# aclyde11/molecular-VAE

Measured on AMD Instinct MI355X. Metric: molecules/s (ELBO fwd+bwd+step), higher is better.
Workload: dtype bf16

## Files before the change

molecular-vae_amd/csrc/gemm.hip:

```cpp
#include "tile_pipe.hpp"
#include "kernels.hpp"
#include <stdlib.h>

struct GemmArgs {
  const void* A; const void* B; void* C; const float* bias; float* partial;
  long lda, ldb, ldc;
  int M, N, K;
  int c_dtype, act, accumulate;
  int tiles_m, tiles_n, splits;
  long kper;
  int a_group, b_group;
  long a_gstride, b_gstride, a_total, b_total;
  float* colsum_out; float* colsum_partial; int colsum_acc; int colsum_nparts; int ones_col;
};
__device__ __forceinline__ long grow(int r, int group, long gstride, long ld) {
  return group > 0 ? (long)(r / group) * gstride + (long)(r % group) * ld : (long)r * ld;
}

__device__ __forceinline__ void store_out(void* C, long off, int c_dtype, float v, int accumulate) {
  if (c_dtype == MVAE_F32) {
    float* p = reinterpret_cast<float*>(C) + off;
    *p = accumulate ? (*p + v) : v;
  } else {
    reinterpret_cast<bf16_t*>(C)[off].x = f2bf(v);
  }
}

__device__ __forceinline__ int xcd_remap(int bid, int n) {
  const int q = n >> 3, r = n & 7, x = bid & 7, i = bid >> 3;
  return (x < r ? x * (q + 1) : r * (q + 1) + (x - r) * q) + i;
}

template <typename T, int BM, int BN, bool PIPE, bool X3 = false>
__global__ __launch_bounds__(256) void gemm_nt_kernel(GemmArgs p) {
  extern __shared__ __attribute__((aligned(16))) char smem[];
  constexpr int WM = BM / 2, WN = BN / 2, MI = WM / 16, NI = WN / 16;
  const int tid = threadIdx.x, lane = tid & 63, wave = tid >> 6, wm = wave >> 1, wn = wave & 1;
  const int ntile = p.tiles_m * p.tiles_n;
  const int tile = xcd_remap(blockIdx.x, ntile);
  const int tm = tile / p.tiles_n, tn = tile - tm * p.tiles_n;
  const int m0 = tm * BM, n0 = tn * BN;
  const int split = blockIdx.y;
  const long kbeg = (long)split * p.kper;
  const long kend = (kbeg + p.kper < (long)p.K) ? (kbeg + p.kper) : (long)p.K;

  const T* A = reinterpret_cast<const T*>(p.A);
  const T* B = reinterpret_cast<const T*>(p.B);
  auto rowA = [&](int r) -> const T* { const int gm = m0 + r; return gm < p.M ? A + grow(gm, p.a_group, p.a_gstride, p.lda) : nullptr; };
  auto rowB = [&](int r) -> const T* { const int gn = n0 + r; return gn < p.N ? B + (long)gn * p.ldb : nullptr; };

  f32x4 acc[MI][NI];
#pragma unroll
  for (int i = 0; i < MI; ++i)
#pragma unroll
    for (int j = 0; j < NI; ++j) acc[i][j] = f32x4{0.f, 0.f, 0.f, 0.f};
  int brow[NI];
#pragma unroll
  for (int j = 0; j < NI; ++j) brow[j] = wn * WN + j * 16;

  if constexpr (PIPE) {
    constexpr int NBUF = 4;
    PipeSeg<BM, BN> s0, s1;
    const uint32_t sz = (uint32_t)sizeof(T);
    auto offA = [&](int r) -> uint32_t { const int gm = m0 + r; return gm < p.M ? (uint32_t)grow(gm, p.a_group, p.a_gstride, p.lda) * sz : PIPE_OOB; };
    auto offB = [&](int r) -> uint32_t { const int gn = n0 + r; return gn < p.N ? (uint32_t)gn * (uint32_t)p.ldb * sz : PIPE_OOB; };
    const uint32_t bytesA = (uint32_t)(p.a_total * sz - kbeg * sz), bytesB = (uint32_t)((long)p.N * p.ldb * sz - kbeg * sz);
    pipe_seg_init<T, BM, BN>(s0, A + kbeg, bytesA, B + kbeg, bytesB, offA, offB, (int)(kend - kbeg), tid);
    s1 = s0; s1.nk = 0;
    tile_gemm_pipe<T, BM, BN, MI, NI, NBUF, NI, 0, X3>(smem, s0, s1, wm * WM, wn * WN, acc, tid);
  } else {
    tile_gemm_segment<T, BM, BN, MI, NI>(smem, rowA, rowB, kbeg, kend, wm * WM, brow, acc, tid);
  }

  const int lr = lane & 15, lq = lane >> 4;
#pragma unroll
  for (int i = 0; i < MI; ++i)
#pragma unroll
    for (int j = 0; j < NI; ++j) {
      const int col = n0 + wn * WN + j * 16 + lr;
      if (col >= p.N) continue;
#pragma unroll
      for (int r = 0; r < 4; ++r) {
        const int row = m0 + wm * WM + i * 16 + lq * 4 + r;
        if (row >= p.M) continue;
        float v = acc[i][j][r];
        if (p.splits > 1) {
          p.partial[((long)split * p.M + row) * p.N + col] = v;
        } else {
          if (p.bias) v += p.bias[col];
          if (p.act == MVAE_ACT_SELU) v = selu_f(v); else if (p.act == MVAE_ACT_RELU) v = fmaxf(v, 0.f);
          store_out(p.C, (long)row * p.ldc + col, p.c_dtype, v, p.accumulate);
        }
      }
    }
}

__global__ __launch_bounds__(256) void gemm_splitk_reduce_kernel(GemmArgs p) {
  const long n = (long)p.M * p.N;
  for (long i = (long)blockIdx.x * 256 + threadIdx.x; i < n; i += (long)gridDim.x * 256) {
    const int row = (int)(i / p.N), col = (int)(i - (long)row * p.N);
    float v = 0.f;
    for (int s = 0; s < p.splits; ++s) v += p.partial[(long)s * n + i];
    if (p.bias) v += p.bias[col];
    if (p.act == MVAE_ACT_SELU) v = selu_f(v); else if (p.act == MVAE_ACT_RELU) v = fmaxf(v, 0.f);
    store_out(p.C, (long)row * p.ldc + col, p.c_dtype, v, p.accumulate);
  }
  if (p.colsum_out && p.colsum_partial) {
    for (long i = (long)blockIdx.x * 256 + threadIdx.x; i < p.M; i += (long)gridDim.x * 256) {
// ... 158 lines not shown
  }
}
struct TnColsumFinish { const float* partial[MVAE_MAX_LAYERS * 2]; float* out[MVAE_MAX_LAYERS * 2]; int M[MVAE_MAX_LAYERS * 2], acc[MVAE_MAX_LAYERS * 2]; int n; };
__global__ __launch_bounds__(256) void gemm_tn_colsum_finish_kernel(TnColsumFinish f) {
  const int gi = blockIdx.y;
  if (gi >= f.n) return;
  for (int i = blockIdx.x * 256 + threadIdx.x; i < f.M[gi]; i += gridDim.x * 256) {
    const float v = f.partial[gi][i] + f.partial[gi][f.M[gi] + i];
    f.out[gi][i] = f.acc[gi] ? f.out[gi][i] + v : v;
  }
}

namespace {
struct Plan { int bm, bn, tiles_m, tiles_n, splits; long kper; };

Plan make_plan(int M, int N, int K, int dtype) {
  Plan pl;
  const int ke = (dtype == MVAE_BF16) ? 64 : 32;
  const long t128 = (long)((M + 127) / 128) * ((N + 127) / 128), t64 = (long)((M + 63) / 64) * ((N + 63) / 64);
  auto eff = [](long t) { return (double)t / (double)(((t + 255) / 256) * 256); };
  pl.bm = (t128 >= 192 && eff(t128) >= 0.8 * eff(t64)) ? 128 : 64;
  pl.bn = pl.bm;
  if (dtype == MVAE_F32 && N <= 32 && M >= 128) { pl.bm = 128; pl.bn = 32; }
  pl.tiles_m = (M + pl.bm - 1) / pl.bm;
  pl.tiles_n = (N + pl.bn - 1) / pl.bn;
  const long tiles = (long)pl.tiles_m * pl.tiles_n;
  long ksteps = (K + ke - 1) / ke;
  if (ksteps < 1) ksteps = 1;
  int splits = 1;
  if (tiles < 128 && ksteps >= 16) {
    splits = (int)((256 + tiles - 1) / tiles);
    const long maxs = ksteps / 8;
    if (splits > maxs) splits = (int)maxs;
    if (splits > 64) splits = 64;
    if (splits < 1) splits = 1;
  }
  long per = (ksteps + splits - 1) / splits;
  splits = (int)((ksteps + per - 1) / per);
  pl.splits = splits;
  pl.kper = per * ke;
  return pl;
}
}

size_t gemm_nt_workspace_bytes(int M, int N, int K, int dtype) {
  if (dtype == MVAE_F32X3) dtype = MVAE_F32;
  Plan pl = make_plan(M, N, K, dtype);
  return pl.splits > 1 ? (size_t)pl.splits * M * N * sizeof(float) : 0;
}

int launch_gemm_nt(int dtype, int M, int N, int K, const void* A, long lda, const void* B, long ldb, void* C, long ldc,
                   int c_dtype, const float* bias, int act, int accumulate, void* ws, size_t ws_bytes, hipStream_t st) {
  return launch_gemm_nt_grouped(dtype, M, N, K, A, lda, 0, 0, (long)M * lda, B, ldb, C, ldc, c_dtype, bias, act, accumulate, ws, ws_bytes, st);
}

int launch_gemm_nt_grouped(int dtype, int M, int N, int K, const void* A, long lda, int a_group, long a_gstride, long a_total,
                           const void* B, long ldb, void* C, long ldc, int c_dtype, const float* bias, int act, int accumulate,
                           void* ws, size_t ws_bytes, hipStream_t st) {
  if (M <= 0 || N <= 0) return MVAE_OK;
  if (K < 0 || !A || !B || !C) return MVAE_ERR_INVALID;
  const bool x3 = dtype == MVAE_F32X3;
  if (x3) dtype = MVAE_F32;
  if (dtype != MVAE_F32 && dtype != MVAE_BF16) return MVAE_ERR_INVALID;
  if (c_dtype != MVAE_F32 && c_dtype != MVAE_BF16) return MVAE_ERR_INVALID;
  if (accumulate && c_dtype != MVAE_F32) return MVAE_ERR_INVALID;
  Plan pl = make_plan(M, N, K, dtype);
  GemmArgs p;
  p.A = A; p.B = B; p.C = C; p.bias = bias; p.partial = nullptr;
  p.lda = lda; p.ldb = ldb; p.ldc = ldc; p.M = M; p.N = N; p.K = K;
  p.c_dtype = c_dtype; p.act = act; p.accumulate = accumulate;
  p.tiles_m = pl.tiles_m; p.tiles_n = pl.tiles_n; p.splits = pl.splits; p.kper = pl.kper;
  p.a_group = a_group; p.a_gstride = a_gstride; p.a_total = a_total; p.b_group = 0; p.b_gstride = 0; p.b_total = (long)N * ldb;
  p.colsum_out = nullptr; p.colsum_partial = nullptr; p.colsum_acc = 0; p.colsum_nparts = 0; p.ones_col = -1;
  if (pl.splits > 1) {
    const size_t need = (size_t)pl.splits * M * N * sizeof(float);
    if (!ws || ws_bytes < need) return MVAE_ERR_WORKSPACE;
    p.partial = reinterpret_cast<float*>(ws);
  }
  dim3 grid(pl.tiles_m * pl.tiles_n, pl.splits), block(256);
  const int sz = (dtype == MVAE_BF16) ? 2 : 4, ke = KB / sz;
  const bool pipe = (K % ke == 0) && (pl.kper % ke == 0) && (lda % (16 / sz) == 0) && (ldb % (16 / sz) == 0) &&
                    ((reinterpret_cast<uintptr_t>(A) | reinterpret_cast<uintptr_t>(B)) % 16 == 0) &&
                    (a_total * sz < (1L << 31)) && ((long)N * ldb * sz < (1L << 31)) && K >= 4 * ke &&
                    (a_group == 0 || a_gstride % (16 / sz) == 0);
  const size_t lds = (size_t)(pipe ? 4 : 2) * (pl.bm + pl.bn) * KB;
#define MVAE_GEMM_LAUNCH2(TT_, BM_, BN_, PIPE_)                                                       \
  do {                                                                                                \
    auto kern = gemm_nt_kernel<TT_, BM_, BN_, PIPE_>;                                                 \
    static bool attr_set = false;                                                                     \
    if (!attr_set) { MVAE_CHECK_HIP(hipFuncSetAttribute(reinterpret_cast<const void*>(kern), hipFuncAttributeMaxDynamicSharedMemorySize, 160 * 1024)); attr_set = true; } \
    hipLaunchKernelGGL(kern, grid, block, lds, st, p);                                                \
  } while (0)
#define MVAE_GEMM_LAUNCH(TT_, BM_, PIPE_) MVAE_GEMM_LAUNCH2(TT_, BM_, BM_, PIPE_)
#define MVAE_GEMM_LAUNCH3(BM_)                                                                        \
  do {                                                                                                \
    auto kern = gemm_nt_kernel<float, BM_, BM_, true, true>;                                          \
    static bool attr_set = false;                                                                     \
    if (!attr_set) { MVAE_CHECK_HIP(hipFuncSetAttribute(reinterpret_cast<const void*>(kern), hipFuncAttributeMaxDynamicSharedMemorySize, 160 * 1024)); attr_set = true; } \
    hipLaunchKernelGGL(kern, grid, block, lds, st, p);                                                \
  } while (0)
  if (pl.bn == 32) {
    if (pipe) MVAE_GEMM_LAUNCH2(float, 128, 32, true); else MVAE_GEMM_LAUNCH2(float, 128, 32, false);
  } else if (dtype == MVAE_BF16) {
    if (pl.bm == 128) { if (pipe) MVAE_GEMM_LAUNCH(bf16_t, 128, true); else MVAE_GEMM_LAUNCH(bf16_t, 128, false); }
    else { if (pipe) MVAE_GEMM_LAUNCH(bf16_t, 64, true); else MVAE_GEMM_LAUNCH(bf16_t, 64, false); }
  } else if (x3 && pipe) {
    if (pl.bm == 128) MVAE_GEMM_LAUNCH3(128); else MVAE_GEMM_LAUNCH3(64);
  } else {
    if (pl.bm == 128) { if (pipe) MVAE_GEMM_LAUNCH(float, 128, true); else MVAE_GEMM_LAUNCH(float, 128, false); }
    else { if (pipe) MVAE_GEMM_LAUNCH(float, 64, true); else MVAE_GEMM_LAUNCH(float, 64, false); }
  }
#undef MVAE_GEMM_LAUNCH
#undef MVAE_GEMM_LAUNCH2
#undef MVAE_GEMM_LAUNCH3
  MVAE_CHECK_HIP(hipGetLastError());
  if (pl.splits > 1) {
    long n = (long)M * N;
    int blocks = (int)((n + 255) / 256);
    if (blocks > 2048) blocks = 2048;
    hipLaunchKernelGGL(gemm_splitk_reduce_kernel, dim3(blocks), block, 0, st, p);
    MVAE_CHECK_HIP(hipGetLastError());
  }
  return MVAE_OK;
}

namespace {
Plan make_plan_tn(int M, int N, int K) {
  Plan pl;
  const char* fe = mvae_knob("MVAE_TN_BM");
  const int force_bm = fe ? atoi(fe) : 0;
// ... 231 lines not shown
    for (int j = 0; j < 2; ++j) {
      const int col = n0 + wn * 32 + j * 16 + lr;
      if (col >= p.N && !(CS && col == p.ones_col)) continue;
#pragma unroll
      for (int r = 0; r < 4; ++r) {
        const int row = m0 + wm * 32 + i * 16 + lq * 4 + r;
        if (row >= p.M) continue;
        const float v = acc[i][j][r];
        if (CS && col == p.ones_col) {
          if (p.splits > 1) p.colsum_partial[(long)split * p.M + row] = v;
          else p.colsum_out[row] = p.colsum_acc ? p.colsum_out[row] + v : v;
        } else if (p.splits > 1) p.partial[((long)split * p.M + row) * p.N + col] = v;
        else store_out(p.C, (long)row * p.ldc + col, p.c_dtype, v, p.accumulate);
      }
    }
}
template <bool X3, bool CS = false>
__global__ __launch_bounds__(256) void gemm_tn_f32_kernel(GemmArgs p) {
  __shared__ float As[2][TNF_KS * TNF_LD];
  __shared__ float Bs[2][TNF_KS * TNF_LD];
  gemm_tn_f32_body<X3, CS>(p, xcd_remap(blockIdx.x, p.tiles_m * p.tiles_n), blockIdx.y, As, Bs);
}

struct TnF32Multi {
  GemmArgs p[MVAE_TN_F32_MULTI_MAX];
  int first[MVAE_TN_F32_MULTI_MAX + 1];
  int flags[MVAE_TN_F32_MULTI_MAX];
  int n;
};
static_assert(sizeof(TnF32Multi) <= 4000, "kernel argument block");
__global__ __launch_bounds__(256) void gemm_tn_f32_multi_kernel(TnF32Multi m) {
  __shared__ float As[2][TNF_KS * TNF_LD];
  __shared__ float Bs[2][TNF_KS * TNF_LD];
  int g = 0;
  while (g + 1 < m.n && (int)blockIdx.x >= m.first[g + 1]) ++g;
  const GemmArgs& p = m.p[g];
  const int local = (int)blockIdx.x - m.first[g], tiles = p.tiles_m * p.tiles_n;
  const int split = local / tiles, tile = local - split * tiles;
  switch (m.flags[g]) {
    case 0: gemm_tn_f32_body<false, false>(p, tile, split, As, Bs); break;
    case 1: gemm_tn_f32_body<true, false>(p, tile, split, As, Bs); break;
    case 2: gemm_tn_f32_body<false, true>(p, tile, split, As, Bs); break;
    default: gemm_tn_f32_body<true, true>(p, tile, split, As, Bs); break;
  }
}
__global__ __launch_bounds__(256) void gemm_splitk_reduce_multi_kernel(TnF32Multi m) {
// ... 16 lines not shown
}

namespace {
Plan make_plan_tn_f32(int M, int N, int R, int target = 768) {
  Plan pl;
  pl.bm = TNF_BM;
  pl.tiles_m = (M + TNF_BM - 1) / TNF_BM; pl.tiles_n = (N + TNF_BM - 1) / TNF_BM;
  const long tiles = (long)pl.tiles_m * pl.tiles_n;
  long steps = (R + TNF_KS - 1) / TNF_KS;
  if (steps < 1) steps = 1;
  int splits = 1;
  if (tiles < (target * 2) / 3 && steps >= 16) {
    splits = (int)((target + tiles - 1) / tiles);
    const long maxs = steps / 8;
    if (splits > maxs) splits = (int)maxs;
    if (splits > 64) splits = 64;
    if (splits < 1) splits = 1;
  }
  const long per = (steps + splits - 1) / splits;
  pl.splits = (int)((steps + per - 1) / per);
  pl.kper = per * TNF_KS;
  return pl;
}
}

size_t gemm_tn_f32_workspace_bytes(int M, int N, int R) {
  Plan pl = make_plan_tn_f32(M, N + 1, R);
  Plan p0 = make_plan_tn_f32(M, N, R);
  const int sp = pl.splits > p0.splits ? pl.splits : p0.splits;
  return sp > 1 ? (size_t)sp * M * (N + 1) * sizeof(float) : 0;
}

int launch_gemm_tn_f32(int M, int N, int R, const float* A, long lda, int a_group, long a_gstride, const float* B, long ldb, int b_group,
                       long b_gstride, float* C, long ldc, int accumulate, void* ws, size_t ws_bytes, hipStream_t st, bool x3,
                       float* colsum_out, int colsum_acc) {
  if (M <= 0 || N <= 0) return MVAE_OK;
  if (R < 0 || !A || !B || !C) return MVAE_ERR_INVALID;
  if ((lda | ldb | a_gstride | b_gstride) & 3) return MVAE_ERR_INVALID;
  if ((reinterpret_cast<uintptr_t>(A) | reinterpret_cast<uintptr_t>(B)) & 15) return MVAE_ERR_INVALID;
  Plan pl = make_plan_tn_f32(M, colsum_out ? N + 1 : N, R);
  GemmArgs p;
  p.A = A; p.B = B; p.C = C; p.bias = nullptr; p.partial = nullptr;
  p.lda = lda; p.ldb = ldb; p.ldc = ldc; p.M = M; p.N = N; p.K = R;
  p.c_dtype = MVAE_F32; p.act = MVAE_ACT_NONE; p.accumulate = accumulate;
  p.tiles_m = pl.tiles_m; p.tiles_n = pl.tiles_n; p.splits = pl.splits; p.kper = pl.kper;
  p.a_group = a_group; p.a_gstride = a_gstride; p.b_group = b_group; p.b_gstride = b_gstride; p.a_total = 0; p.b_total = 0;
  p.colsum_out = colsum_out; p.colsum_partial = nullptr; p.colsum_acc = colsum_acc; p.colsum_nparts = pl.splits; p.ones_col = colsum_out ? N : -1;
  if (pl.splits > 1) {
    const size_t need = (size_t)pl.splits * M * (N + (colsum_out ? 1 : 0)) * sizeof(float);
    if (!ws || ws_bytes < need) return MVAE_ERR_WORKSPACE;
    p.partial = reinterpret_cast<float*>(ws);
    if (colsum_out) p.colsum_partial = p.partial + (size_t)pl.splits * M * N;
  }
  const dim3 tgrid(pl.tiles_m * pl.tiles_n, pl.splits);
  if (colsum_out) {
    if (x3) hipLaunchKernelGGL((gemm_tn_f32_kernel<true, true>), tgrid, dim3(256), 0, st, p);
    else hipLaunchKernelGGL((gemm_tn_f32_kernel<false, true>), tgrid, dim3(256), 0, st, p);
  } else {
    if (x3) hipLaunchKernelGGL((gemm_tn_f32_kernel<true, false>), tgrid, dim3(256), 0, st, p);
    else hipLaunchKernelGGL((gemm_tn_f32_kernel<false, false>), tgrid, dim3(256), 0, st, p);
  }
  MVAE_CHECK_HIP(hipGetLastError());
  if (pl.splits > 1) {
    long n = (long)M * N;
    int blocks = (int)((n + 255) / 256);
    if (blocks > 2048) blocks = 2048;
    hipLaunchKernelGGL(gemm_splitk_reduce_kernel, dim3(blocks), dim3(256), 0, st, p);
    MVAE_CHECK_HIP(hipGetLastError());
  }
  return MVAE_OK;
}


namespace {
int tnf_multi_target(int n) { int t = 1536 / (n > 0 ? n : 1); return t < 96 ? 96 : (t > 768 ? 768 : t); }
Plan tnf_multi_plan(const mvae_gemm_tn_f32_problem& q, int n) { return make_plan_tn_f32(q.M, q.colsum_out ? q.N + 1 : q.N, (int)q.K, tnf_multi_target(n)); }
size_t tnf_multi_need(const mvae_gemm_tn_f32_problem& q, const Plan& pl) {
  return pl.splits > 1 ? (((size_t)pl.splits * q.M * (q.N + (q.colsum_out ? 1 : 0)) * sizeof(float) + 255) & ~(size_t)255) : 0;
}
}
extern "C" size_t mvae_gemm_tn_f32_multi_workspace(int n, const mvae_gemm_tn_f32_problem* pr) {
  if (n < 1 || n > MVAE_TN_F32_MULTI_MAX || !pr) return 0;
  size_t b = 0;
  for (int i = 0; i < n; ++i) if (pr[i].M > 0 && pr[i].N > 0 && pr[i].K >= 0 && pr[i].K < (1L << 31)) b += tnf_multi_need(pr[i], tnf_multi_plan(pr[i], n));
  return b;
}
extern "C" int mvae_gemm_tn_f32_multi(int n, const mvae_gemm_tn_f32_problem* pr, void* ws, size_t ws_bytes, void* stream) {
  if (n < 1 || n > MVAE_TN_F32_MULTI_MAX || !pr) return MVAE_ERR_INVALID;
  if (mvae_gemm_tn_f32_multi_workspace(n, pr) > ws_bytes || (mvae_gemm_tn_f32_multi_workspace(n, pr) && !ws)) return MVAE_ERR_WORKSPACE;
  TnF32Multi m;
  m.n = n;
  char* wsp = reinterpret_cast<char*>(ws);
  int blocks = 0, any_split = 0;
  long max_mn = 1;
  for (int i = 0; i < n; ++i) {
    const mvae_gemm_tn_f32_problem& q = pr[i];
    if (q.M < 1 || q.N < 1 || q.K < 0 || q.K >= (1L << 31) || !q.A || !q.B || !q.C) return MVAE_ERR_INVALID;
    if ((q.lda | q.ldb | q.a_gstride | q.b_gstride) & 3) return MVAE_ERR_INVALID;
    if ((reinterpret_cast<uintptr_t>(q.A) | reinterpret_cast<uintptr_t>(q.B)) & 15) return MVAE_ERR_INVALID;
    const Plan pl = tnf_multi_plan(q, n);
    GemmArgs& p = m.p[i];
    p.A = q.A; p.B = q.B; p.C = q.C; p.bias = nullptr; p.partial = nullptr;
    p.lda = q.lda; p.ldb = q.ldb; p.ldc = q.ldc; p.M = q.M; p.N = q.N; p.K = (int)q.K;
    p.c_dtype = MVAE_F32; p.act = MVAE_ACT_NONE; p.accumulate = q.accumulate;
    p.tiles_m = pl.tiles_m; p.tiles_n = pl.tiles_n; p.splits = pl.splits; p.kper = pl.kper;
    p.a_group = q.a_group; p.a_gstride = q.a_gstride; p.b_group = q.b_group; p.b_gstride = q.b_gstride; p.a_total = 0; p.b_total = 0;
    p.colsum_out = q.colsum_out; p.colsum_partial = nullptr; p.colsum_acc = q.colsum_accumulate; p.colsum_nparts = pl.splits; p.ones_col = q.colsum_out ? q.N : -1;
    if (pl.splits > 1) {
      p.partial = reinterpret_cast<float*>(wsp);
      if (q.colsum_out) p.colsum_partial = p.partial + (size_t)pl.splits * q.M * q.N;
      wsp += tnf_multi_need(q, pl);
      any_split = 1;
// ... 76 lines not shown
```

molecular-vae_amd/csrc/tile_pipe.hpp:

```cpp
#pragma once
#include <type_traits>
#include "tile.hpp"

constexpr uint32_t PIPE_OOB = 0x80000000u;

template <int BM, int BN, int NT = 256> struct PipeSeg {
  __amdgpu_buffer_rsrc_t ra, rb;
  uint32_t offA[BM * 8 / NT];
  uint32_t offB[BN * 8 / NT];
  int nk;
  int hole_st; uint32_t hole_bytes;
};

template <typename T, int BM, int BN, int NT = 256, typename RowOffA, typename RowOffB>
__device__ __forceinline__ void pipe_seg_init(PipeSeg<BM, BN, NT>& s, const void* A, uint32_t bytesA, const void* B, uint32_t bytesB,
                                              RowOffA rowoffA, RowOffB rowoffB, int K, int tid) {
  constexpr int KE = KB / (int)sizeof(T);
  s.ra = __builtin_amdgcn_make_buffer_rsrc(const_cast<void*>(A), 0, (int)bytesA, 0x00020000);
  s.rb = __builtin_amdgcn_make_buffer_rsrc(const_cast<void*>(B), 0, (int)bytesB, 0x00020000);
  s.nk = (A != nullptr) ? K / KE : 0;
  s.hole_st = 0x7fffffff; s.hole_bytes = 0;
#pragma unroll
  for (int i = 0; i < BM * 8 / NT; ++i) {
    const int id = tid + i * NT, row = id >> 3, pos = id & 7;
// ... 39 lines not shown
};
template <int N, int JS, int BOUT> struct FragReadB<N, N, JS, BOUT> {
  static __device__ __forceinline__ void run(u32x4 (&)[N], uint32_t) {}
};
template <int N> __device__ __forceinline__ void wait_lgkmcnt() {
  __builtin_amdgcn_sched_barrier(0);
  asm volatile("s_waitcnt lgkmcnt(%0)" ::"n"(N) : "memory");
  __builtin_amdgcn_sched_barrier(0);
}

__device__ __forceinline__ void split_x3(const u32x4& c0, const u32x4& c1, uint4& hi, uint4& lo) {
  const uint32_t x[8] = {c0[0], c0[1], c0[2], c0[3], c1[0], c1[1], c1[2], c1[3]};
  uint32_t h[4], l[4];
#pragma unroll
  for (int j = 0; j < 4; ++j) {
    const uint32_t h0 = x[2 * j] & 0xffff0000u, h1 = x[2 * j + 1] & 0xffff0000u;
    const float l0 = __builtin_bit_cast(float, x[2 * j]) - __builtin_bit_cast(float, h0);
    const float l1 = __builtin_bit_cast(float, x[2 * j + 1]) - __builtin_bit_cast(float, h1);
    h[j] = (h0 >> 16) | h1;
    l[j] = (uint32_t)f2bf(l0) | ((uint32_t)f2bf(l1) << 16);
  }
  hi = make_uint4(h[0], h[1], h[2], h[3]); lo = make_uint4(l[0], l[1], l[2], l[3]);
}
template <int MI, int NI, int JS, int BOUT>
__device__ __forceinline__ void tile_mma_asm_x3(uint32_t a_base, uint32_t b_base, const uint32_t (&a_lane)[2], const uint32_t (&b_lane)[2],
                                                f32x4 (&acc)[MI][NI]) {
  u32x4 a0[MI], b0[NI], a1[MI], b1[NI];
  FragRead<0, MI, 16 * KB>::run(a0, a_base + a_lane[0]);
  FragReadB<0, NI, JS, BOUT>::run(b0, b_base + b_lane[0]);
  FragRead<0, MI, 16 * KB>::run(a1, a_base + a_lane[1]);
  FragReadB<0, NI, JS, BOUT>::run(b1, b_base + b_lane[1]);
  wait_lgkmcnt<0>();
  uint4 ah[MI], al[MI], bh[NI], bl[NI];
#pragma unroll
  for (int mi = 0; mi < MI; ++mi) split_x3(a0[mi], a1[mi], ah[mi], al[mi]);
#pragma unroll
  for (int ni = 0; ni < NI; ++ni) split_x3(b0[ni], b1[ni], bh[ni], bl[ni]);
#pragma unroll
  for (int mi = 0; mi < MI; ++mi)
#pragma unroll
    for (int ni = 0; ni < NI; ++ni) {
      mma16<bf16_t>(al[mi], bh[ni], acc[mi][ni]);
      mma16<bf16_t>(ah[mi], bl[ni], acc[mi][ni]);
      mma16<bf16_t>(ah[mi], bh[ni], acc[mi][ni]);
    }
}

template <typename T, int MI, int NI, int JS, int BOUT>
__device__ __forceinline__ void tile_mma_asm(uint32_t a_base, uint32_t b_base, const uint32_t (&a_lane)[2], const uint32_t (&b_lane)[2],
                                             f32x4 (&acc)[MI][NI]) {
  u32x4 a0[MI], b0[NI], a1[MI], b1[NI];
  FragRead<0, MI, 16 * KB>::run(a0, a_base + a_lane[0]);
  FragReadB<0, NI, JS, BOUT>::run(b0, b_base + b_lane[0]);
  FragRead<0, MI, 16 * KB>::run(a1, a_base + a_lane[1]);
  FragReadB<0, NI, JS, BOUT>::run(b1, b_base + b_lane[1]);
  wait_lgkmcnt<(MI + NI) < 16 ? (MI + NI) : 15>();
#pragma unroll
  for (int mi = 0; mi < MI; ++mi)
#pragma unroll
    for (int ni = 0; ni < NI; ++ni)
      mma16<T>(__builtin_bit_cast(uint4, a0[mi]), __builtin_bit_cast(uint4, b0[ni]), acc[mi][ni]);
  wait_lgkmcnt<0>();
#pragma unroll
  for (int mi = 0; mi < MI; ++mi)
#pragma unroll
    for (int ni = 0; ni < NI; ++ni)
      mma16<T>(__builtin_bit_cast(uint4, a1[mi]), __builtin_bit_cast(uint4, b1[ni]), acc[mi][ni]);
}

__device__ __forceinline__ void ws_barrier() {
// ... 4 lines not shown
}

template <int BM, int BN, int NBUF, int NT = 256>
__device__ __forceinline__ void pipe_issue_stage(char* smem, const PipeSeg<BM, BN, NT>& s0, const PipeSeg<BM, BN, NT>& s1, int st, int wave) {
#if defined(__HIP_DEVICE_COMPILE__)
  char* stage = smem + (st % NBUF) * ((BM + BN) * KB);
  const bool first = st < s0.nk;
  const PipeSeg<BM, BN, NT>& s = first ? s0 : s1;
  const int ls = first ? st : st - s0.nk;
  const uint32_t kbyte = (uint32_t)ls * KB + (ls >= s.hole_st ? s.hole_bytes : 0u);
#pragma unroll
  for (int i = 0; i < BM * 8 / NT; ++i) {
    lds_void_t* dst = (lds_void_t*)(stage + (i * NT + wave * 64) * 16);
    __builtin_amdgcn_raw_ptr_buffer_load_lds(s.ra, dst, 16, s.offA[i] + kbyte, 0, 0, 0);
  }
#pragma unroll
  for (int i = 0; i < BN * 8 / NT; ++i) {
    lds_void_t* dst = (lds_void_t*)(stage + BM * KB + (i * NT + wave * 64) * 16);
    __builtin_amdgcn_raw_ptr_buffer_load_lds(s.rb, dst, 16, s.offB[i] + kbyte, 0, 0, 0);
  }
#endif
}

template <typename T, int BM, int BN, int MI, int NI, int NBUF, int JS, int BOUT, bool X3 = false>
__device__ __forceinline__ void tile_gemm_pipe(char* smem, const PipeSeg<BM, BN>& s0, const PipeSeg<BM, BN>& s1, int arow0,
                                               int brow0, f32x4 (&acc)[MI][NI], int tid) {
  static_assert(!X3 || std::is_same<T, float>::value, "the 3 x bf16 product form takes fp32 operands");
  constexpr int STAGE = (BM + BN) * KB;
  constexpr int LPS = (BM + BN) * 8 / 256;
  static_assert((NBUF - 2) * LPS < 64, "vmcnt range");
  static_assert((BM + BN) * 8 % 256 == 0 && BM * 8 % 256 == 0, "whole LDS-DMA pieces per thread");
  const int lane = tid & 63;
  const int wave = __builtin_amdgcn_readfirstlane(tid >> 6);
  const int nk = s0.nk + s1.nk;
  if (nk <= 0) return;
  const uint32_t lds0 = (uint32_t)(uintptr_t)(lds_void_t*)smem;
  const int lr = lane & 15, lk = lane >> 4;
  uint32_t a_lane[2], b_lane[2];
#pragma unroll
  for (int kk = 0; kk < 2; ++kk) {
    a_lane[kk] = (uint32_t)swz(arow0 + lr, kk * 4 + lk);
    b_lane[kk] = (uint32_t)swz(brow0 + lr, kk * 4 + lk) + BM * KB;
  }
#pragma unroll
  for (int s = 0; s < NBUF - 1; ++s)
    if (s < nk) pipe_issue_stage<BM, BN, NBUF>(smem, s0, s1, s, wave);
  for (int kt = 0; kt < nk; ++kt) {
    if (kt + NBUF - 2 < nk) wait_vmcnt<(NBUF - 2) * LPS>();
    else wait_vmcnt<0>();
    __builtin_amdgcn_s_barrier();
    asm volatile("" ::: "memory");
    if (kt + NBUF - 1 < nk) pipe_issue_stage<BM, BN, NBUF>(smem, s0, s1, kt + NBUF - 1, wave);
    const uint32_t st = lds0 + (uint32_t)((kt % NBUF) * STAGE);
    if constexpr (X3) tile_mma_asm_x3<MI, NI, JS, BOUT>(st, st, a_lane, b_lane, acc);
    else tile_mma_asm<T, MI, NI, JS, BOUT>(st, st, a_lane, b_lane, acc);
  }
  __builtin_amdgcn_s_barrier();
}


__device__ __forceinline__ void SB() { __builtin_amdgcn_sched_barrier(0); }

template <typename T, int MI, int NI, int M0, int M1>
__device__ __forceinline__ void mma_rows(const u32x4 (&a)[MI], const u32x4 (&b)[NI], f32x4 (&acc)[MI][NI]) {
#pragma unroll
  for (int mi = M0; mi < M1; ++mi)
#pragma unroll
    for (int ni = 0; ni < NI; ++ni)
      mma16<T>(__builtin_bit_cast(uint4, a[mi]), __builtin_bit_cast(uint4, b[ni]), acc[mi][ni]);
}

template <typename T, int BM, int BN, int NBUF, int NT, int MI, int NI, int GA, int M0>
__device__ __forceinline__ void pipe_block_with_refill(char* smem, const PipeSeg<BM, BN, NT>& s0, const PipeSeg<BM, BN, NT>& s1, bool refill, int st,
                                                       int wave, const u32x4 (&a)[GA], const u32x4 (&b)[NI], f32x4 (&acc)[MI][NI]) {
  if (refill) pipe_issue_stage<BM, BN, NBUF, NT>(smem, s0, s1, st, wave);
  SB();
#pragma unroll
  for (int r = 0; r < GA; ++r)
// ... 457 lines not shown
    FragReadTN<0, 4, 512>::template run<0>(b0, addrB, st);
    if constexpr (COLSUM) FragReadTN<0, 1, 512>::template run<0>(as, addrS, st);
    __builtin_amdgcn_sched_barrier(0);
    asm volatile("" ::: "memory");
    if (kt + 1 < nk) pipe_tn2_issue(smem, s, kt + 1, wave);
    wait_lgkmcnt<0>();
    TnIlv<0>::run(a0, b0, acc, lo, hi, addrA, addrB, st);
    if constexpr (COLSUM) {
      if (cs_half >= 0) mma16<bf16_t>(__builtin_bit_cast(uint4, as[0]), ones, accb);
    }
    wait_lgkmcnt<0>();
#pragma unroll
    for (int i = 0; i < 8; ++i) a1[i] = u32x4{lo[i][0], lo[i][1], hi[i][0], hi[i][1]};
#pragma unroll
    for (int i = 0; i < 4; ++i) b1[i] = u32x4{lo[8 + i][0], lo[8 + i][1], hi[8 + i][0], hi[8 + i][1]};
#pragma unroll
    for (int mi = 0; mi < 8; ++mi)
#pragma unroll
      for (int ni = 0; ni < 4; ++ni)
        mma16<bf16_t>(__builtin_bit_cast(uint4, a1[mi]), __builtin_bit_cast(uint4, b1[ni]), acc[mi][ni]);
  }
  ws_barrier();
}
```

Baseline: 36090.

## Pre-split fp32 operands into bf16 hi/lo in LDS for x3 GEMMs

Adds dedicated x3 (3×bf16-emulated fp32) GEMM kernels for the NT and TN paths. Each fp32 tile is split once into bf16 hi/lo halves as it is stored to LDS, replacing the per-fragment split that ran inside the MMA loop. This moves split work out of the inner loop and lets fragments be read directly as bf16. The cost is register-staged global loads instead of LDS-DMA pipelining, double LDS buffering only, and new tile-size heuristics, including a cost model that picks between 64 and 128 rows. A single-problem multi TN call is also routed to the new kernel.

Result: faster. 36570, median of 6 (+1.3%).

```diff
diff --git a/molecular-vae_amd/csrc/gemm.hip b/molecular-vae_amd/csrc/gemm.hip
--- a/molecular-vae_amd/csrc/gemm.hip
+++ b/molecular-vae_amd/csrc/gemm.hip
@@ -31,7 +31,7 @@
   return (x < r ? x * (q + 1) : r * (q + 1) + (x - r) * q) + i;
 }
 
-template <typename T, int BM, int BN, bool PIPE, bool X3 = false>
+template <typename T, int BM, int BN, bool PIPE>
 __global__ __launch_bounds__(256) void gemm_nt_kernel(GemmArgs p) {
   extern __shared__ __attribute__((aligned(16))) char smem[];
   constexpr int WM = BM / 2, WN = BN / 2, MI = WM / 16, NI = WN / 16;
@@ -67,7 +67,7 @@
     const uint32_t bytesA = (uint32_t)(p.a_total * sz - kbeg * sz), bytesB = (uint32_t)((long)p.N * p.ldb * sz - kbeg * sz);
     pipe_seg_init<T, BM, BN>(s0, A + kbeg, bytesA, B + kbeg, bytesB, offA, offB, (int)(kend - kbeg), tid);
     s1 = s0; s1.nk = 0;
-    tile_gemm_pipe<T, BM, BN, MI, NI, NBUF, NI, 0, X3>(smem, s0, s1, wm * WM, wn * WN, acc, tid);
+    tile_gemm_pipe<T, BM, BN, MI, NI, NBUF, NI, 0>(smem, s0, s1, wm * WM, wn * WN, acc, tid);
   } else {
     tile_gemm_segment<T, BM, BN, MI, NI>(smem, rowA, rowB, kbeg, kend, wm * WM, brow, acc, tid);
   }
@@ -84,6 +84,116 @@
         const int row = m0 + wm * WM + i * 16 + lq * 4 + r;
         if (row >= p.M) continue;
         float v = acc[i][j][r];
+        if (p.splits > 1) {
+          p.partial[((long)split * p.M + row) * p.N + col] = v;
+        } else {
+          if (p.bias) v += p.bias[col];
+          if (p.act == MVAE_ACT_SELU) v = selu_f(v); else if (p.act == MVAE_ACT_RELU) v = fmaxf(v, 0.f);
+          store_out(p.C, (long)row * p.ldc + col, p.c_dtype, v, p.accumulate);
+        }
+      }
+    }
+}
+
+template <int BM, int BN>
+__global__ __launch_bounds__(256, BM == 64 ? 3 : 2) void gemm_nt_x3_kernel(GemmArgs p) {
+  extern __shared__ __attribute__((aligned(16))) char smem[];
+  constexpr int WM = BM / 2, WN = BN / 2, MI = WM / 16, NI = WN / 16, NA = BM / 16, NB = BN / 16;
+  constexpr int A_HI = 0, A_LO = BM * KB, B_HI = 2 * BM * KB, B_LO = 2 * BM * KB + BN * KB;
+  const int tid = threadIdx.x, lane = tid & 63, wave = tid >> 6, wm = wave >> 1, wn = wave & 1;
+  const int tile = xcd_remap(blockIdx.x, p.tiles_m * p.tiles_n);
+  const int tm = tile / p.tiles_n, tn = tile - tm * p.tiles_n;
+  const int m0 = tm * BM, n0 = tn * BN;
+  const int split = blockIdx.y;
+  const long kbeg = (long)split * p.kper;
+  const long kend = (kbeg + p.kper < (long)p.K) ? (kbeg + p.kper) : (long)p.K;
+  const float* A = reinterpret_cast<const float*>(p.A);
+  const float* B = reinterpret_cast<const float*>(p.B);
+  const int j = tid & 15, r16 = tid >> 4;
+  const int jc = (j >> 3) * 4 + (j & 3), jh = ((j >> 2) & 1) * 8;
+  uint32_t offa[NA], offb[NB];
+#pragma unroll
+  for (int i = 0; i < NA; ++i) { const int gm = m0 + r16 + 16 * i; offa[i] = gm < p.M ? (uint32_t)grow(gm, p.a_group, p.a_gstride, p.lda) : 0u; }
+#pragma unroll
+  for (int i = 0; i < NB; ++i) { const int gn = n0 + r16 + 16 * i; offb[i] = gn < p.N ? (uint32_t)((long)gn * p.ldb) : 0u; }
+  float4 va[NA], vb[NB];
+  bool kin = true;
+  auto load_stage = [&](long k0) {
+    kin = k0 + 4 * j < kend;
+    const long k = kin ? k0 + 4 * j : kbeg;
+#pragma unroll
+    for (int i = 0; i < NA; ++i) va[i] = *reinterpret_cast<const float4*>(A + offa[i] + k);
+#pragma unroll
+    for (int i = 0; i < NB; ++i) vb[i] = *reinterpret_cast<const float4*>(B + offb[i] + k);
+  };
+  auto store_stage = [&]() {
+    if (!kin) {
+#pragma unroll
+      for (int i = 0; i < NA; ++i) va[i] = make_float4(0.f, 0.f, 0.f, 0.f);
+#pragma unroll
+      for (int i = 0; i < NB; ++i) vb[i] = make_float4(0.f, 0.f, 0.f, 0.f);
+    }
+#pragma unroll
+    for (int i = 0; i < NA; ++i) {
+      uint2 hi, lo;
+      split_x3_4(va[i], hi, lo);
+      char* d = smem + swz(r16 + 16 * i, jc) + jh;
+      *reinterpret_cast<uint2*>(d + A_HI) = hi;
+      *reinterpret_cast<uint2*>(d + A_LO) = lo;
+    }
+#pragma unroll
+    for (int i = 0; i < NB; ++i) {
+      uint2 hi, lo;
+      split_x3_4(vb[i], hi, lo);
+      char* d = smem + swz(r16 + 16 * i, jc) + jh;
+      *reinterpret_cast<uint2*>(d + B_HI) = hi;
+      *reinterpret_cast<uint2*>(d + B_LO) = lo;
+    }
+  };
+  f32x4 acc[MI][NI];
+#pragma unroll
+  for (int i = 0; i < MI; ++i)
+#pragma unroll
+    for (int jj = 0; jj < NI; ++jj) acc[i][jj] = f32x4{0.f, 0.f, 0.f, 0.f};
+  const int lr = lane & 15, lq = lane >> 4;
+  const int nst = (int)((kend - kbeg + 63) / 64);
+  if (nst > 0) {
+    load_stage(kbeg);
+    store_stage();
+    for (int s = 0; s < nst; ++s) {
+      __syncthreads();
+      if (s + 1 < nst) load_stage(kbeg + (long)(s + 1) * 64);
+      u32x4 ah[MI], al[MI], bh[NI], bl[NI];
+#pragma unroll
+      for (int kk = 0; kk < 2; ++kk) {
+        const int chunk = kk * 4 + lq;
+#pragma unroll
+        for (int mi = 0; mi < MI; ++mi) {
+          const char* s_ = smem + swz(wm * WM + mi * 16 + lr, chunk);
+          ah[mi] = *reinterpret_cast<const u32x4*>(s_ + A_HI); al[mi] = *reinterpret_cast<const u32x4*>(s_ + A_LO);
+        }
+#pragma unroll
+        for (int ni = 0; ni < NI; ++ni) {
+          const char* s_ = smem + swz(wn * WN + ni * 16 + lr, chunk);
+          bh[ni] = *reinterpret_cast<const u32x4*>(s_ + B_HI); bl[ni] = *reinterpret_cast<const u32x4*>(s_ + B_LO);
+        }
+        if (kk == 1) __syncthreads();
+        mma_x3_block<MI, NI>(ah, al, bh, bl, acc);
+      }
+      if (s + 1 < nst) store_stage();
+    }
+  }
+#pragma unroll
+  for (int i = 0; i < MI; ++i)
+#pragma unroll
+    for (int jj = 0; jj < NI; ++jj) {
+      const int col = n0 + wn * WN + jj * 16 + lr;
+      if (col >= p.N) continue;
+#pragma unroll
+      for (int r = 0; r < 4; ++r) {
+        const int row = m0 + wm * WM + i * 16 + lq * 4 + r;
+        if (row >= p.M) continue;
+        float v = acc[i][jj][r];
         if (p.splits > 1) {
           p.partial[((long)split * p.M + row) * p.N + col] = v;
         } else {
@@ -288,6 +398,17 @@
   pl.bm = (t128 >= 192 && eff(t128) >= 0.8 * eff(t64)) ? 128 : 64;
   pl.bn = pl.bm;
   if (dtype == MVAE_F32 && N <= 32 && M >= 128) { pl.bm = 128; pl.bn = 32; }
+  if (dtype == MVAE_F32X3) {
+    pl.bm = 128; pl.bn = N <= 64 ? 64 : 128;
+    const long tiles128 = (long)((M + 127) / 128) * ((N + pl.bn - 1) / pl.bn), tiles64 = (long)((M + 63) / 64) * ((N + pl.bn - 1) / pl.bn);
+    const double cost128 = (double)((tiles128 + 511) / 512) * 2 * 128, cost64 = (double)((tiles64 + 767) / 768) * 3 * 64 * 1.15;
+    if (pl.bn == 128 && tiles128 > 512 && cost64 < cost128) pl.bm = 64;
+    const Plan pf = make_plan(M, N, K, MVAE_F32);
+    pl.tiles_m = (M + pl.bm - 1) / pl.bm;
+    pl.tiles_n = (N + pl.bn - 1) / pl.bn;
+    pl.splits = pf.splits; pl.kper = pf.kper;
+    return pl;
+  }
   pl.tiles_m = (M + pl.bm - 1) / pl.bm;
   pl.tiles_n = (N + pl.bn - 1) / pl.bn;
   const long tiles = (long)pl.tiles_m * pl.tiles_n;
@@ -330,7 +451,15 @@
   if (dtype != MVAE_F32 && dtype != MVAE_BF16) return MVAE_ERR_INVALID;
   if (c_dtype != MVAE_F32 && c_dtype != MVAE_BF16) return MVAE_ERR_INVALID;
   if (accumulate && c_dtype != MVAE_F32) return MVAE_ERR_INVALID;
-  Plan pl = make_plan(M, N, K, dtype);
+  const int sz = (dtype == MVAE_BF16) ? 2 : 4, ke = KB / sz;
+  const bool pipe = (K % ke == 0) && (lda % (16 / sz) == 0) && (ldb % (16 / sz) == 0) &&
+                    ((reinterpret_cast<uintptr_t>(A) | reinterpret_cast<uintptr_t>(B)) % 16 == 0) &&
+                    (a_total * sz < (1L << 31)) && ((long)N * ldb * sz < (1L << 31)) && K >= 4 * ke &&
+                    (a_group == 0 || a_gstride % (16 / sz) == 0);
+  const bool x3k = x3 && (K % 4 == 0) && (lda % 4 == 0) && (ldb % 4 == 0) && ((reinterpret_cast<uintptr_t>(A) | reinterpret_cast<uintptr_t>(B)) % 16 == 0) &&
+                   (a_total * 4 < (1L << 31)) && ((long)N * ldb * 4 < (1L << 31)) && K >= 4 * ke && (a_group == 0 || a_gstride % 4 == 0) &&
+                   !(N <= 32 && M >= 128);
+  Plan pl = make_plan(M, N, K, x3k ? MVAE_F32X3 : dtype);
   GemmArgs p;
   p.A = A; p.B = B; p.C = C; p.bias = bias; p.partial = nullptr;
   p.lda = lda; p.ldb = ldb; p.ldc = ldc; p.M = M; p.N = N; p.K = K;
@@ -344,12 +473,7 @@
     p.partial = reinterpret_cast<float*>(ws);
   }
   dim3 grid(pl.tiles_m * pl.tiles_n, pl.splits), block(256);
-  const int sz = (dtype == MVAE_BF16) ? 2 : 4, ke = KB / sz;
-  const bool pipe = (K % ke == 0) && (pl.kper % ke == 0) && (lda % (16 / sz) == 0) && (ldb % (16 / sz) == 0) &&
-                    ((reinterpret_cast<uintptr_t>(A) | reinterpret_cast<uintptr_t>(B)) % 16 == 0) &&
-                    (a_total * sz < (1L << 31)) && ((long)N * ldb * sz < (1L << 31)) && K >= 4 * ke &&
-                    (a_group == 0 || a_gstride % (16 / sz) == 0);
-  const size_t lds = (size_t)(pipe ? 4 : 2) * (pl.bm + pl.bn) * KB;
+  const size_t lds = (size_t)(x3k ? 2 : pipe ? 4 : 2) * (pl.bm + pl.bn) * KB;
 #define MVAE_GEMM_LAUNCH2(TT_, BM_, BN_, PIPE_)                                                       \
   do {                                                                                                \
     auto kern = gemm_nt_kernel<TT_, BM_, BN_, PIPE_>;                                                 \
@@ -358,9 +482,9 @@
     hipLaunchKernelGGL(kern, grid, block, lds, st, p);                                                \
   } while (0)
 #define MVAE_GEMM_LAUNCH(TT_, BM_, PIPE_) MVAE_GEMM_LAUNCH2(TT_, BM_, BM_, PIPE_)
-#define MVAE_GEMM_LAUNCH3(BM_)                                                                        \
+#define MVAE_GEMM_LAUNCH3(BM_, BN_)                                                                   \
   do {                                                                                                \
-    auto kern = gemm_nt_kernel<float, BM_, BM_, true, true>;                                          \
+    auto kern = gemm_nt_x3_kernel<BM_, BN_>;                                                          \
     static bool attr_set = false;                                                                     \
     if (!attr_set) { MVAE_CHECK_HIP(hipFuncSetAttribute(reinterpret_cast<const void*>(kern), hipFuncAttributeMaxDynamicSharedMemorySize, 160 * 1024)); attr_set = true; } \
     hipLaunchKernelGGL(kern, grid, block, lds, st, p);                                                \
@@ -370,8 +494,8 @@
   } else if (dtype == MVAE_BF16) {
     if (pl.bm == 128) { if (pipe) MVAE_GEMM_LAUNCH(bf16_t, 128, true); else MVAE_GEMM_LAUNCH(bf16_t, 128, false); }
     else { if (pipe) MVAE_GEMM_LAUNCH(bf16_t, 64, true); else MVAE_GEMM_LAUNCH(bf16_t, 64, false); }
-  } else if (x3 && pipe) {
-    if (pl.bm == 128) MVAE_GEMM_LAUNCH3(128); else MVAE_GEMM_LAUNCH3(64);
+  } else if (x3k) {
+    if (pl.bn == 64) MVAE_GEMM_LAUNCH3(128, 64); else if (pl.bm == 64) MVAE_GEMM_LAUNCH3(64, 128); else MVAE_GEMM_LAUNCH3(128, 128);
   } else {
     if (pl.bm == 128) { if (pipe) MVAE_GEMM_LAUNCH(float, 128, true); else MVAE_GEMM_LAUNCH(float, 128, false); }
     else { if (pipe) MVAE_GEMM_LAUNCH(float, 64, true); else MVAE_GEMM_LAUNCH(float, 64, false); }
@@ -649,6 +773,151 @@
   gemm_tn_f32_body<X3, CS>(p, xcd_remap(blockIdx.x, p.tiles_m * p.tiles_n), blockIdx.y, As, Bs);
 }
 
+constexpr int TNX_KS = 64;
+__device__ __forceinline__ int tnx_slot(int r) { return (r & 32) | ((r & 3) << 3) | ((r >> 2) & 7); }
+template <int WGM, int NI, bool CS>
+__global__ __launch_bounds__(256, 2) void gemm_tn_x3_kernel(GemmArgs p) {
+  extern __shared__ __attribute__((aligned(16))) char smem[];
+  constexpr int BM = 64 * WGM, WN = 16 * NI, BN = (4 / WGM) * WN;
+  constexpr int RA = BM * 2, RB = BN * 2;
+  constexpr int PA = TNX_KS * RA, PB = TNX_KS * RB;
+  constexpr int CPA = BM / 4, RPA = 256 / CPA, NA = TNX_KS / RPA;
+  constexpr int CPB = BN / 4, RPB = 256 / CPB, NB = TNX_KS / RPB;
+  const int tid = threadIdx.x, lane = tid & 63, wave = tid >> 6;
+  const int wm = WGM == 2 ? (wave >> 1) : 0, wn = WGM == 2 ? (wave & 1) : wave;
+  const int tile = xcd_remap(blockIdx.x, p.tiles_m * p.tiles_n);
+  const int tm = tile / p.tiles_n, tn = tile - tm * p.tiles_n;
+  const int m0 = tm * BM, n0 = tn * BN;
+  const int split = blockIdx.y;
+  const long rbeg = (long)split * p.kper;
+  const long rend = (rbeg + p.kper < (long)p.K) ? (rbeg + p.kper) : (long)p.K;
+  const float* A = reinterpret_cast<const float*>(p.A);
+  const float* B = reinterpret_cast<const float*>(p.B);
+  const int ca = (tid % CPA) * 4, ka = tid / CPA, cb = (tid % CPB) * 4, kb = tid / CPB;
+  const bool a_in = m0 + ca < p.M, b_in = n0 + cb < p.N;
+  const bool b_one = CS && n0 + cb == p.ones_col;
+  long oa, ob; int ia, ib;
+  auto row_init = [&](long r, int group, long gstride, long ld, long& off, int& in_g) {
+    if (group > 0) { const long qg = r / group; in_g = (int)(r - qg * group); off = qg * gstride + (long)in_g * ld; }
+    else { in_g = 0; off = r * ld; }
+  };
+  auto row_step = [&](int rows, int group, long gstride, long ld, long& off, int& in_g) {
+    off += (long)rows * ld;
+    if (group > 0) { in_g += rows; while (in_g >= group) { in_g -= group; off += gstride - (long)group * ld; } }
+  };
+  row_init(rbeg + ka, p.a_group, p.a_gstride, p.lda, oa, ia);
+  row_init(rbeg + kb, p.b_group, p.b_gstride, p.ldb, ob, ib);
+  float4 va[NA], vb[NB];
+  const int cola = a_in ? m0 + ca : 0, colb = b_in ? n0 + cb : 0;
+  const int nrow = (int)(rend - rbeg);
+  int rpend = 0;
+  auto load_stage = [&](int r0) {
+    rpend = r0;
+#pragma unroll
+    for (int i = 0; i < NA; ++i) {
+      va[i] = *reinterpret_cast<const float4*>(r0 + ka + i * RPA < nrow ? A + oa + cola : A);
+      row_step(RPA, p.a_group, p.a_gstride, p.lda, oa, ia);
+    }
+#pragma unroll
+    for (int i = 0; i < NB; ++i) {
+      vb[i] = *reinterpret_cast<const float4*>(r0 + kb + i * RPB < nrow ? B + ob + colb : B);
+      row_step(RPB, p.b_group, p.b_gstride, p.ldb, ob, ib);
+    }
+  };
+  auto store_stage = [&]() {
+    if constexpr (CS) {
+      if (b_one) {
+#pragma unroll
+        for (int i = 0; i < NB; ++i) vb[i].x = 1.f;
+      }
+    }
+    if (rpend + TNX_KS > nrow) {
+#pragma unroll
+      for (int i = 0; i < NA; ++i) if (rpend + ka + i * RPA >= nrow) va[i] = make_float4(0.f, 0.f, 0.f, 0.f);
+#pragma unroll
+      for (int i = 0; i < NB; ++i) if (rpend + kb + i * RPB >= nrow) vb[i] = make_float4(0.f, 0.f, 0.f, 0.f);
+    }
+#pragma unroll
+    for (int i = 0; i < NA; ++i) {
+      const int kr = tnx_slot(ka + i * RPA);
+      uint2 hi, lo;
+      split_x3_4(va[i], hi, lo);
+      char* d = smem + kr * RA + ((((uint32_t)(ca >> 4)) ^ tnx_f<RA>(kr)) << 5) + (ca & 15) * 2;
+      *reinterpret_cast<uint2*>(d) = hi;
+      *reinterpret_cast<uint2*>(d + PA) = lo;
+    }
+#pragma unroll
+    for (int i = 0; i < NB; ++i) {
+      const int kr = tnx_slot(kb + i * RPB);
+      uint2 hi, lo;
+      split_x3_4(vb[i], hi, lo);
+      char* d = smem + 2 * PA + kr * RB + ((((uint32_t)(cb >> 4)) ^ tnx_f<RB>(kr)) << 5) + (cb & 15) * 2;
+      *reinterpret_cast<uint2*>(d) = hi;
+      *reinterpret_cast<uint2*>(d + PB) = lo;
+    }
+  };
+  f32x4 acc[4][NI];
+#pragma unroll
+  for (int i = 0; i < 4; ++i)
+#pragma unroll
+    for (int j = 0; j < NI; ++j) acc[i][j] = f32x4{0.f, 0.f, 0.f, 0.f};
+  const int nst = (int)((rend - rbeg + TNX_KS - 1) / TNX_KS);
+  if (nst > 0) {
+    const uint32_t lds0 = (uint32_t)(uintptr_t)(lds_void_t*)smem;
+    const int g = lane >> 4, q = (lane >> 2) & 3, pp = lane & 3;
+    uint32_t addrA[4], addrB[NI];
+#pragma unroll
+    for (int i = 0; i < 4; ++i)
+      addrA[i] = (uint32_t)(8 * g + q) * (uint32_t)RA + ((((uint32_t)(wm * 4 + i)) ^ tnx_f<RA>(8 * g + q)) << 5) + (uint32_t)pp * 8u;
+#pragma unroll
+    for (int i = 0; i < NI; ++i)
+      addrB[i] = (uint32_t)(8 * g + q) * (uint32_t)RB + ((((uint32_t)(wn * NI + i)) ^ tnx_f<RB>(8 * g + q)) << 5) + (uint32_t)pp * 8u + 2u * PA;
+    u32x4 ah[4], al[4], bh[NI], bl[NI];
+    load_stage(0);
+    store_stage();
+    for (int s = 0; s < nst; ++s) {
+      __syncthreads();
+      asm volatile("" ::: "memory");
+      if (s + 1 < nst) load_stage((s + 1) * TNX_KS);
+      FragReadTN<0, 4, RA>::template run<0>(ah, addrA, lds0);
+      FragReadTN<0, NI, RB>::template run<0>(bh, addrB, lds0);
+      FragReadTN<0, 4, RA>::template run<0>(al, addrA, lds0 + PA);
+      FragReadTN<0, NI, RB>::template run<0>(bl, addrB, lds0 + PB);
+      wait_lgkmcnt<0>();
+      mma_x3_block<4, NI>(ah, al, bh, bl, acc);
+      __builtin_amdgcn_sched_barrier(0);
+      FragReadTN<0, 4, RA>::template run<32 * RA>(ah, addrA, lds0);
+      FragReadTN<0, NI, RB>::template run<32 * RB>(bh, addrB, lds0);
+      FragReadTN<0, 4, RA>::template run<32 * RA>(al, addrA, lds0 + PA);
+      FragReadTN<0, NI, RB>::template run<32 * RB>(bl, addrB, lds0 + PB);
+      wait_lgkmcnt<0>();
+      __syncthreads();
+      asm volatile("" ::: "memory");
+      mma_x3_block<4, NI>(ah, al, bh, bl, acc);
+      if (s + 1 < nst) store_stage();
+    }
+  }
+  const int lr = lane & 15, lq = lane >> 4;
+#pragma unroll
+  for (int i = 0; i < 4; ++i)
+#pragma unroll
+    for (int j = 0; j < NI; ++j) {
+      const int col = n0 + wn * WN + j * 16 + lr;
+      if (col >= p.N && !(CS && col == p.ones_col)) continue;
+#pragma unroll
+      for (int r = 0; r < 4; ++r) {
+        const int row = m0 + wm * 64 + i * 16 + lq * 4 + r;
+        if (row >= p.M) continue;
+        const float v = acc[i][j][r];
+        if (CS && col == p.ones_col) {
+          if (p.splits > 1) p.colsum_partial[(long)split * p.M + row] = v;
+          else p.colsum_out[row] = p.colsum_acc ? p.colsum_out[row] + v : v;
+        } else if (p.splits > 1) p.partial[((long)split * p.M + row) * p.N + col] = v;
+        else store_out(p.C, (long)row * p.ldc + col, p.c_dtype, v, p.accumulate);
+      }
+    }
+}
+
 struct TnF32Multi {
   GemmArgs p[MVAE_TN_F32_MULTI_MAX];
   int first[MVAE_TN_F32_MULTI_MAX + 1];
@@ -711,6 +980,13 @@
   pl.kper = per * TNF_KS;
   return pl;
 }
+Plan make_plan_tn_x3(int M, int N, int R) {
+  Plan pl = make_plan_tn_f32(M, N, R);
+  pl.bm = 64; pl.bn = 128;
+  pl.tiles_m = (M + pl.bm - 1) / pl.bm; pl.tiles_n = (N + pl.bn - 1) / pl.bn;
+  return pl;
+}
+bool tn_x3_takes(int M, int N) { return M % 4 == 0 && N % 4 == 0; }
 }
 
 size_t gemm_tn_f32_workspace_bytes(int M, int N, int R) {
@@ -727,7 +1003,8 @@
   if (R < 0 || !A || !B || !C) return MVAE_ERR_INVALID;
   if ((lda | ldb | a_gstride | b_gstride) & 3) return MVAE_ERR_INVALID;
   if ((reinterpret_cast<uintptr_t>(A) | reinterpret_cast<uintptr_t>(B)) & 15) return MVAE_ERR_INVALID;
-  Plan pl = make_plan_tn_f32(M, colsum_out ? N + 1 : N, R);
+  const bool x3k = x3 && tn_x3_takes(M, N);
+  Plan pl = x3k ? make_plan_tn_x3(M, colsum_out ? N + 1 : N, R) : make_plan_tn_f32(M, colsum_out ? N + 1 : N, R);
   GemmArgs p;
   p.A = A; p.B = B; p.C = C; p.bias = nullptr; p.partial = nullptr;
   p.lda = lda; p.ldb = ldb; p.ldc = ldc; p.M = M; p.N = N; p.K = R;
@@ -742,7 +1019,17 @@
     if (colsum_out) p.colsum_partial = p.partial + (size_t)pl.splits * M * N;
   }
   const dim3 tgrid(pl.tiles_m * pl.tiles_n, pl.splits);
-  if (colsum_out) {
+  if (x3k) {
+    static bool attr_set = false;
+    if (!attr_set) {
+      MVAE_CHECK_HIP(hipFuncSetAttribute(reinterpret_cast<const void*>(gemm_tn_x3_kernel<1, 2, false>), hipFuncAttributeMaxDynamicSharedMemorySize, 160 * 1024));
+      MVAE_CHECK_HIP(hipFuncSetAttribute(reinterpret_cast<const void*>(gemm_tn_x3_kernel<1, 2, true>), hipFuncAttributeMaxDynamicSharedMemorySize, 160 * 1024));
+      attr_set = true;
+    }
+    const size_t lds = (size_t)2 * TNX_KS * 2 * (pl.bm + pl.bn);
+    if (colsum_out) hipLaunchKernelGGL((gemm_tn_x3_kernel<1, 2, true>), tgrid, dim3(256), lds, st, p);
+    else hipLaunchKernelGGL((gemm_tn_x3_kernel<1, 2, false>), tgrid, dim3(256), lds, st, p);
+  } else if (colsum_out) {
     if (x3) hipLaunchKernelGGL((gemm_tn_f32_kernel<true, true>), tgrid, dim3(256), 0, st, p);
     else hipLaunchKernelGGL((gemm_tn_f32_kernel<false, true>), tgrid, dim3(256), 0, st, p);
   } else {
@@ -767,6 +1054,9 @@
 size_t tnf_multi_need(const mvae_gemm_tn_f32_problem& q, const Plan& pl) {
   return pl.splits > 1 ? (((size_t)pl.splits * q.M * (q.N + (q.colsum_out ? 1 : 0)) * sizeof(float) + 255) & ~(size_t)255) : 0;
 }
+bool tnf_multi_single_x3(int n, const mvae_gemm_tn_f32_problem* pr) {
+  return n == 1 && pr[0].x3 && pr[0].M > 0 && pr[0].N > 0 && pr[0].K >= 0 && pr[0].K < (1L << 31) && tn_x3_takes(pr[0].M, pr[0].N);
+}
 }
 extern "C" size_t mvae_gemm_tn_f32_multi_workspace(int n, const mvae_gemm_tn_f32_problem* pr) {
   if (n < 1 || n > MVAE_TN_F32_MULTI_MAX || !pr) return 0;
@@ -777,6 +1067,12 @@
 extern "C" int mvae_gemm_tn_f32_multi(int n, const mvae_gemm_tn_f32_problem* pr, void* ws, size_t ws_bytes, void* stream) {
   if (n < 1 || n > MVAE_TN_F32_MULTI_MAX || !pr) return MVAE_ERR_INVALID;
   if (mvae_gemm_tn_f32_multi_workspace(n, pr) > ws_bytes || (mvae_gemm_tn_f32_multi_workspace(n, pr) && !ws)) return MVAE_ERR_WORKSPACE;
+  if (tnf_multi_single_x3(n, pr)) {
+    const mvae_gemm_tn_f32_problem& q = pr[0];
+    if (!q.A || !q.B || !q.C) return MVAE_ERR_INVALID;
+    return launch_gemm_tn_f32(q.M, q.N, (int)q.K, q.A, q.lda, q.a_group, q.a_gstride, q.B, q.ldb, q.b_group, q.b_gstride, q.C, q.ldc, q.accumulate,
+                              ws, ws_bytes, (hipStream_t)stream, true, q.colsum_out, q.colsum_accumulate);
+  }
   TnF32Multi m;
   m.n = n;
   char* wsp = reinterpret_cast<char*>(ws);
diff --git a/molecular-vae_amd/csrc/tile_pipe.hpp b/molecular-vae_amd/csrc/tile_pipe.hpp
--- a/molecular-vae_amd/csrc/tile_pipe.hpp
+++ b/molecular-vae_amd/csrc/tile_pipe.hpp
@@ -85,30 +85,6 @@
   }
   hi = make_uint4(h[0], h[1], h[2], h[3]); lo = make_uint4(l[0], l[1], l[2], l[3]);
 }
-template <int MI, int NI, int JS, int BOUT>
-__device__ __forceinline__ void tile_mma_asm_x3(uint32_t a_base, uint32_t b_base, const uint32_t (&a_lane)[2], const uint32_t (&b_lane)[2],
-                                                f32x4 (&acc)[MI][NI]) {
-  u32x4 a0[MI], b0[NI], a1[MI], b1[NI];
-  FragRead<0, MI, 16 * KB>::run(a0, a_base + a_lane[0]);
-  FragReadB<0, NI, JS, BOUT>::run(b0, b_base + b_lane[0]);
-  FragRead<0, MI, 16 * KB>::run(a1, a_base + a_lane[1]);
-  FragReadB<0, NI, JS, BOUT>::run(b1, b_base + b_lane[1]);
-  wait_lgkmcnt<0>();
-  uint4 ah[MI], al[MI], bh[NI], bl[NI];
-#pragma unroll
-  for (int mi = 0; mi < MI; ++mi) split_x3(a0[mi], a1[mi], ah[mi], al[mi]);
-#pragma unroll
-  for (int ni = 0; ni < NI; ++ni) split_x3(b0[ni], b1[ni], bh[ni], bl[ni]);
-#pragma unroll
-  for (int mi = 0; mi < MI; ++mi)
-#pragma unroll
-    for (int ni = 0; ni < NI; ++ni) {
-      mma16<bf16_t>(al[mi], bh[ni], acc[mi][ni]);
-      mma16<bf16_t>(ah[mi], bl[ni], acc[mi][ni]);
-      mma16<bf16_t>(ah[mi], bh[ni], acc[mi][ni]);
-    }
-}
-
 template <typename T, int MI, int NI, int JS, int BOUT>
 __device__ __forceinline__ void tile_mma_asm(uint32_t a_base, uint32_t b_base, const uint32_t (&a_lane)[2], const uint32_t (&b_lane)[2],
                                              f32x4 (&acc)[MI][NI]) {
@@ -159,10 +135,9 @@
 #endif
 }
 
-template <typename T, int BM, int BN, int MI, int NI, int NBUF, int JS, int BOUT, bool X3 = false>
+template <typename T, int BM, int BN, int MI, int NI, int NBUF, int JS, int BOUT>
 __device__ __forceinline__ void tile_gemm_pipe(char* smem, const PipeSeg<BM, BN>& s0, const PipeSeg<BM, BN>& s1, int arow0,
                                                int brow0, f32x4 (&acc)[MI][NI], int tid) {
-  static_assert(!X3 || std::is_same<T, float>::value, "the 3 x bf16 product form takes fp32 operands");
   constexpr int STAGE = (BM + BN) * KB;
   constexpr int LPS = (BM + BN) * 8 / 256;
   static_assert((NBUF - 2) * LPS < 64, "vmcnt range");
@@ -189,8 +164,7 @@
     asm volatile("" ::: "memory");
     if (kt + NBUF - 1 < nk) pipe_issue_stage<BM, BN, NBUF>(smem, s0, s1, kt + NBUF - 1, wave);
     const uint32_t st = lds0 + (uint32_t)((kt % NBUF) * STAGE);
-    if constexpr (X3) tile_mma_asm_x3<MI, NI, JS, BOUT>(st, st, a_lane, b_lane, acc);
-    else tile_mma_asm<T, MI, NI, JS, BOUT>(st, st, a_lane, b_lane, acc);
+    tile_mma_asm<T, MI, NI, JS, BOUT>(st, st, a_lane, b_lane, acc);
   }
   __builtin_amdgcn_s_barrier();
 }
@@ -694,3 +668,32 @@
   }
   ws_barrier();
 }
+
+__device__ __forceinline__ void split_x3_4(const float4& v, uint2& hi, uint2& lo) {
+  const uint32_t h0 = __builtin_bit_cast(uint32_t, v.x) & 0xffff0000u, h1 = __builtin_bit_cast(uint32_t, v.y) & 0xffff0000u;
+  const uint32_t h2 = __builtin_bit_cast(uint32_t, v.z) & 0xffff0000u, h3 = __builtin_bit_cast(uint32_t, v.w) & 0xffff0000u;
+  const float l0 = v.x - __builtin_bit_cast(float, h0), l1 = v.y - __builtin_bit_cast(float, h1);
+  const float l2 = v.z - __builtin_bit_cast(float, h2), l3 = v.w - __builtin_bit_cast(float, h3);
+  hi = make_uint2((h0 >> 16) | h1, (h2 >> 16) | h3);
+  typedef float f32x2_t __attribute__((ext_vector_type(2)));
+  typedef __bf16 bf16x2_t __attribute__((ext_vector_type(2)));
+  lo = make_uint2(__builtin_bit_cast(uint32_t, __builtin_convertvector((f32x2_t){l0, l1}, bf16x2_t)),
+                  __builtin_bit_cast(uint32_t, __builtin_convertvector((f32x2_t){l2, l3}, bf16x2_t)));
+}
+template <int MI, int NI>
+__device__ __forceinline__ void mma_x3_block(const u32x4 (&ah)[MI], const u32x4 (&al)[MI], const u32x4 (&bh)[NI], const u32x4 (&bl)[NI],
+                                             f32x4 (&acc)[MI][NI]) {
+#pragma unroll
+  for (int mi = 0; mi < MI; ++mi)
+#pragma unroll
+    for (int ni = 0; ni < NI; ++ni) {
+      mma16<bf16_t>(__builtin_bit_cast(uint4, al[mi]), __builtin_bit_cast(uint4, bh[ni]), acc[mi][ni]);
+      mma16<bf16_t>(__builtin_bit_cast(uint4, ah[mi]), __builtin_bit_cast(uint4, bl[ni]), acc[mi][ni]);
+      mma16<bf16_t>(__builtin_bit_cast(uint4, ah[mi]), __builtin_bit_cast(uint4, bh[ni]), acc[mi][ni]);
+    }
+}
+template <int ROWB> __device__ __forceinline__ uint32_t tnx_f(int krow) {
+  static_assert(ROWB == 128 || ROWB % 256 == 0, "row length");
+  if constexpr (ROWB == 128) return (uint32_t)(((krow >> 1) & 1) | (((krow >> 3) & 1) << 1));
+  else return tn_f(krow);
+}
```
